# Mehooz/vision4leg

Measured on AMD Instinct MI355X. Metric: PPO env-steps/s (encoder+update, sim excluded), higher is better.
Workload: dtype f16; 1 GPU; ppo_locotransformer thin-goal: LocoTransformer S=93 A=6, E=32 envs x T=512, B=1024, 3 opt epochs; net=loco, envs_per_gpu=32, horizon=512, minibatch=1024, opt_epochs=3, parallelism=dp1, includes_rollout_inference=True, logp_old=recorded at action time (target_pf forward skipped; SURVEY 8d declared saving)

## Files before the change

### vision4leg_amd/csrc/bwd.h

```cpp
#pragma once
#include "infer.h"

namespace v4l {

struct BwdLayer {
  const void *w2t, *w1t, *wot, *wint;
  const float *g1, *g2;
  const float* dy;
  const float *s_qkv, *s_P, *s_xh1, *s_rs1, *s_xh2, *s_rs2;
  const void* s_f;
  void *o_dz2, *o_df, *o_dz1, *o_dqkv;
  float* o_dx;
  float *gp2, *bp2, *gp1, *bp1;
};

struct BwdLayerStack { BwdLayer l[2]; };

struct BwdHead {
  const void *w2t, *w1t, *w0t;
  const float* dout;
  const float *s_h1, *s_h0;
  float *o_dh1, *o_dh0;
};
struct BwdTail {
  const void *wpt, *wf2t, *wupt;
  const float* x0;
  const float *s_e1, *s_e0;
  const float* s_c3;
  float *o_dhc, *o_de0;
  float* o_dc3;
};

template <typename T, int SPW> struct BwdLayLds {
  static constexpr int ROWS = InfRows<SPW>::ROWS;
// ... 656 lines not shown
#pragma unroll
      for (int j = 0; j < 4; ++j) {
        const int n4 = nt4[j] * 16 + qr;
        const float d0 = m[j].x > 0.f ? acc[0][j][0] : 0.f, d1 = m[j].y > 0.f ? acc[0][j][1] : 0.f;
        const float d2 = m[j].z > 0.f ? acc[0][j][2] : 0.f, d3 = m[j].w > 0.f ? acc[0][j][3] : 0.f;
        if (dst != nullptr) st4(dst + fr * LY::LDF + n4, d0, d1, d2, d3);
        if (ok) st4(save + (int64_t)(s0 + fr) * 256 + n4, d0, d1, d2, d3);
      }
    };
    zero_acc(acc);
    block_gemm<T, 1, 4, 2>(acc, dt, LY::LDX, (const T*)tl.wpt, 64, nt4, lane, ring_pr);
    masked(tm_e1, dh, tl.o_dhc);
    __syncthreads();
    zero_acc(acc);
    block_gemm<T, 1, 4, 8>(acc, dh, LY::LDF, (const T*)tl.wf2t, 256, nt4, lane, ring_f2);
    masked(tm_e0, (T*)nullptr, tl.o_de0);
  }
  LAY_STAMP(9);
}


struct BwdConv {
  const void* w3d;
  const void* w2d[4];
  const void* image;
  const int* rowidx;
  const float *c1, *c2;
  const float* dc3;
  float *slab1, *slab2, *slab3;
  float *bslab1, *bslab2, *bslab3;
  int n;
  void *t_dc2, *t_dc1;
};
template <typename T> struct BwdConvLds {
  static constexpr bool B16 = sizeof(T) == 2;
  static constexpr int LF = 64 + 4;
  static constexpr int LC1 = 32 + (B16 ? 8 : 0);
  static constexpr int IMGP = B16 ? 1 : 2;
  static constexpr int LT = 64 + (B16 ? 8 : 4);
  static constexpr int LP2 = 64 + (B16 ? 8 : 4);
  static constexpr int LP1 = 256 + (B16 ? 8 : 4);
  static constexpr size_t dc3_b = (size_t)17 * LT * sizeof(T);
  static constexpr size_t c2_b = (size_t)36 * LF * 4;
  static constexpr size_t dc2_b = (size_t)48 * LT * sizeof(T);
  static constexpr size_t dc2T_b = (size_t)64 * LP2 * sizeof(T);
  static constexpr size_t c1_b = ((size_t)225 * LC1 * sizeof(T) + 15) / 16 * 16;
  static constexpr size_t dc1_b = (size_t)32 * LP1 * sizeof(T);
  static constexpr size_t img_b = (size_t)(4 / IMGP) * 4096 * sizeof(T);
  static constexpr size_t w2_b = B16 ? (size_t)4 * 32 * 256 * sizeof(T) : 0;
  static constexpr size_t bytes = dc3_b + c2_b + dc2_b + dc2T_b + c1_b + dc1_b + img_b + w2_b;
  static_assert(bytes <= 160 * 1024, "one block per CU");
};

template <typename T> __device__ __forceinline__ typename Frag<T>::type frag_of(const float (&v)[8]) {
  typename Frag<T>::type f;
  if constexpr (sizeof(T) == 2) {
#pragma unroll
    for (int j = 0; j < 8; ++j) f[j] = (T)v[j];
  } else {
#pragma unroll
    for (int j = 0; j < 8; ++j) f.v[j] = v[j];
  }
  return f;
}
template <typename H>
__device__ __forceinline__ typename Frag<H>::type frag_of_t(const H (&v)[8]) {
  static_assert(sizeof(H) == 2, "16-bit operand type");
  typename Frag<H>::type f;
#pragma unroll
  for (int j = 0; j < 8; ++j) f[j] = v[j];
  return f;
}
__device__ __forceinline__ f32x8 frag_of_t(const float (&v)[8]) { return frag_of<float>(v); }

template <typename T, int MT, int NT, int KS, int KS0 = 0, int PDEPTH = 4, class RowF>
__device__ __forceinline__ void gather_gemm(f32x4 (&acc)[MT][NT], const T* __restrict__ W, int Kp, int nt0, int lane, RowF arow) {
  typedef typename Frag<T>::type frag_t;
  constexpr int PD = NT >= 2 ? 2 : (KS < PDEPTH ? KS : PDEPTH);
  const int fr = lane & 15, fg = (lane >> 4) * 8;
  const T* wrow = W + (int64_t)(nt0 * 16 + fr) * Kp + fg + KS0 * 32;
  frag_t fb[PD][NT];
#pragma unroll
  for (int d = 0; d < PD; ++d)
#pragma unroll
    for (int j = 0; j < NT; ++j) fb[d][j] = *reinterpret_cast<const frag_t*>(wrow + (int64_t)j * 16 * Kp + d * 32);
#pragma unroll
  for (int ks = 0; ks < KS; ++ks) {
    frag_t cur[NT];
#pragma unroll
    for (int j = 0; j < NT; ++j) cur[j] = fb[ks % PD][j];
    if (ks + PD < KS) {
#pragma unroll
      for (int j = 0; j < NT; ++j) fb[ks % PD][j] = *reinterpret_cast<const frag_t*>(wrow + (int64_t)j * 16 * Kp + (ks + PD) * 32);
    }
#pragma unroll
    for (int mt = 0; mt < MT; ++mt) {
      const frag_t fa = *reinterpret_cast<const frag_t*>(arow(mt, (ks + KS0) >> 1) + ((ks + KS0) & 1) * 32 + fg);
#pragma unroll
      for (int j = 0; j < NT; ++j)
        mma_k32(acc[mt][j], cur[j], fa);
    }
  }
}

#ifdef V4L_INFER_TIMING
#define CONV_STAMP(i) do { if (blockIdx.x == 0 && threadIdx.x == 0 && smp == 3 * (int)gridDim.x) g_inf_stamps[16 + (i)] = clock64(); } while (0)
#else
#define CONV_STAMP(i)
#endif
template <typename T, bool A16 = false>
__global__ __launch_bounds__(512) void bwd_conv_kernel(BwdConv a) {
  static_assert(!A16 || sizeof(T) == 2, "A16: activations saved in the bf16 operand type");
  typedef BwdConvLds<T> LY;
  typedef typename Frag<T>::type frag_t;
  constexpr int NTH = 512;
  extern __shared__ __attribute__((aligned(16))) unsigned char smem[];
  T* sdc3 = reinterpret_cast<T*>(smem);
  float* sc2 = reinterpret_cast<float*>(smem + LY::dc3_b);
  T* sdc2t = reinterpret_cast<T*>(smem + LY::dc3_b + LY::c2_b);
  T* sdc2T = reinterpret_cast<T*>(smem + LY::dc3_b + LY::c2_b + LY::dc2_b);
  constexpr size_t o_c1 = LY::dc3_b + LY::c2_b + LY::dc2_b + LY::dc2T_b;
  T* sc1 = reinterpret_cast<T*>(smem + o_c1);
  T* sdc1T = reinterpret_cast<T*>(smem + o_c1 + LY::c1_b);
  T* simg = reinterpret_cast<T*>(smem + o_c1 + LY::c1_b + LY::dc1_b);
  T* sw2 = reinterpret_cast<T*>(smem + o_c1 + LY::c1_b + LY::dc1_b + LY::img_b);
  const int tid = threadIdx.x, lane = tid & 63, wave = tid >> 6;
  const int fr = lane & 15, g = lane >> 4, qr = g * 4;
  const int kt2 = wave * 4;
  const int ch1 = wave >> 1, th1 = wave & 1;
  f32x4 acc2[4][4], acc1[2][2];
#pragma unroll
  for (int t = 0; t < 4; ++t) {
#pragma unroll
    for (int c = 0; c < 4; ++c) acc2[t][c] = f32x4{0.f, 0.f, 0.f, 0.f};
    acc1[t >> 1][t & 1] = f32x4{0.f, 0.f, 0.f, 0.f};
  }
  float b2r[4] = {0.f, 0.f, 0.f, 0.f};
  float b1r[4] = {0.f, 0.f, 0.f, 0.f};
  for (int i = tid; i < 12 * LY::LT; i += NTH) sdc2t[36 * LY::LT + i] = (T)0.f;
  for (int i = tid; i < 64 * LY::LP2; i += NTH) sdc2T[i] = (T)0.f;
  for (int i = tid; i < 32 * LY::LP1; i += NTH) sdc1T[i] = (T)0.f;
  for (int i = tid; i < LY::LT; i += NTH) sdc3[16 * LY::LT + i] = (T)0.f;
  constexpr int CH = 4 / LY::IMGP;

  constexpr int V = 16 / sizeof(T);
  constexpr int N4 = 225 * 8, PT = (N4 + NTH - 1) / NTH;
  constexpr int N8 = 225 * 4, PT8 = (N8 + NTH - 1) / NTH;
  typedef typename Frag<T>::type chunk_t;
  float4 hv0 = float4{0.f, 0.f, 0.f, 0.f}, hv1 = hv0, cv[A16 ? 1 : PT];
  chunk_t h16 = {}, c16[A16 ? PT8 : 1] = {};
  auto load_next = [&](int sm) {
    const float* g3 = a.dc3 + (int64_t)sm * 16 * 64;
    if constexpr (A16) {
      const chunk_t* g2 = reinterpret_cast<const chunk_t*>(reinterpret_cast<const T*>(a.c2) + (int64_t)sm * 36 * 64);
      const chunk_t* g1 = reinterpret_cast<const chunk_t*>(reinterpret_cast<const T*>(a.c1) + (int64_t)sm * 225 * 32);
      h16 = g2[tid < 288 ? tid : 0];
      if (tid >= 256) hv1 = *reinterpret_cast<const float4*>(g3 + (tid - 256) * 4);
#pragma unroll
      for (int k = 0; k < PT8; ++k) {
        const int i8 = tid + k * NTH;
        c16[k] = g1[i8 < N8 ? i8 : 0];
      }
    } else {
      const float* g2 = a.c2 + (int64_t)sm * 36 * 64;
      const float* g1 = a.c1 + (int64_t)sm * 225 * 32;
      hv0 = *reinterpret_cast<const float4*>(g2 + tid * 4);
      if (tid >= 256) hv1 = *reinterpret_cast<const float4*>(g3 + (tid - 256) * 4);
      else if (tid < 64) hv1 = *reinterpret_cast<const float4*>(g2 + (512 + tid) * 4);
#pragma unroll
      for (int k = 0; k < PT; ++k) {
        const int i4 = tid + k * NTH;
        cv[k] = *reinterpret_cast<const float4*>(g1 + (i4 < N4 ? i4 : 0) * 4);
      }
    }
// ... 57 lines not shown
        const int px = m * 16 + fr;
        okr[m] = px < 36;
        iy[m] = px / 6; ix[m] = px - iy[m] * 6;
      }
      f32x4 acc[3][1];
#pragma unroll
      for (int m = 0; m < 3; ++m) acc[m][0] = f32x4{0.f, 0.f, 0.f, 0.f};
      auto arow = [&](int m, int tap) -> const T* {
        const int ta = tap / 3, tb = tap - ta * 3;
        const int oy = iy[m] - ta, ox = ix[m] - tb;
        const bool ok = okr[m] && oy >= 0 && oy < 4 && ox >= 0 && ox < 4;
        return sdc3 + (ok ? oy * 4 + ox : 16) * LY::LT;
      };
      float4* part = reinterpret_cast<float4*>(simg);
      if (wave >= 4) {
        gather_gemm<T, 3, 1, 9, 9, LY::B16 ? 9 : 3>(acc, W, 576, nt, lane, arow);
#pragma unroll
        for (int m = 0; m < 3; ++m) part[(nt * 3 + m) * 64 + lane] = float4{acc[m][0][0], acc[m][0][1], acc[m][0][2], acc[m][0][3]};
      } else {
        gather_gemm<T, 3, 1, 9, 0, LY::B16 ? 9 : 3>(acc, W, 576, nt, lane, arow);
      }
      __syncthreads();
      if (wave < 4) {
#pragma unroll
        for (int m = 0; m < 3; ++m) {
          const int px = m * 16 + fr, c4 = nt * 16 + qr;
          if (px < 36) {
            const float4 hi = part[(nt * 3 + m) * 64 + lane];
            const float4 mk = *reinterpret_cast<const float4*>(sc2 + px * LY::LF + c4);
            const float d0 = mk.x > 0.f ? acc[m][0][0] + hi.x : 0.f, d1 = mk.y > 0.f ? acc[m][0][1] + hi.y : 0.f;
            const float d2 = mk.z > 0.f ? acc[m][0][2] + hi.z : 0.f, d3 = mk.w > 0.f ? acc[m][0][3] + hi.w : 0.f;
            st4(sdc2t + px * LY::LT + c4, d0, d1, d2, d3);
            if (a.t_dc2 != nullptr) st4(reinterpret_cast<T*>(a.t_dc2) + ((int64_t)smp * 36 + px) * 64 + c4, d0, d1, d2, d3);
            T* tp = sdc2T + c4 * LY::LP2 + px;
            tp[0] = (T)d0; tp[LY::LP2] = (T)d1; tp[2 * LY::LP2] = (T)d2; tp[3 * LY::LP2] = (T)d3;
            b2r[0] += d0; b2r[1] += d1; b2r[2] += d2; b2r[3] += d3;
          }
        }
      }
    }
    __syncthreads();
    CONV_STAMP(2);
#pragma unroll
    for (int k = 0; k < CH * 4096 / V / NTH; ++k)
      __builtin_amdgcn_global_load_lds((const V4L_GLOBAL void*)(gimg + (int64_t)(tid + k * NTH) * V),
                                       (__attribute__((address_space(3))) void*)(simg + ((tid & ~63) + k * NTH) * V), 16, 0, 0);
#pragma unroll
    for (int st = 0; st < 2; ++st) {
      frag_t fy[4];
#pragma unroll
      for (int c = 0; c < 4; ++c) fy[c] = *reinterpret_cast<const frag_t*>(sdc2T + (c * 16 + fr) * LY::LP2 + st * 32 + g * 8);
#pragma unroll
      for (int t = 0; t < 4; ++t) {
        const int kt = kt2 + t, tap = kt >> 1, ci = (kt & 1) * 16 + fr;
        const int ky = tap >> 2, kx = tap & 3;
        T w[8];
#pragma unroll
        for (int j = 0; j < 8; ++j) {
          const int pos = st * 32 + g * 8 + j;
          const int pp = pos < 36 ? pos : 0, oy = pp / 6, ox = pp - oy * 6;
          w[j] = sc1[((2 * oy + ky) * 15 + 2 * ox + kx) * LY::LC1 + ci];
        }
        const frag_t fx = frag_of_t(w);
#pragma unroll
        for (int c = 0; c < 4; ++c) mma_k32(acc2[t][c], fx, fy[c]);
      }
    }
    CONV_STAMP(3);
    {
      const int cls = wave >> 1, py = cls >> 1, pxx = cls & 1, nh = wave & 1;
      const int nIy = (15 - py + 1) >> 1, nIx = (15 - pxx + 1) >> 1;
      int ry[4], rx[4];
#pragma unroll
      for (int m = 0; m < 4; ++m) { const int r = m * 16 + fr; ry[m] = r >> 3; rx[m] = r & 7; }
      f32x4 acc[4][1];
#pragma unroll
      for (int m = 0; m < 4; ++m) acc[m][0] = f32x4{0.f, 0.f, 0.f, 0.f};
      auto arow = [&](int m, int tap) -> const T* {
        const int oy = ry[m] - (tap >> 1), ox = rx[m] - (tap & 1);
        const bool ok = ry[m] < nIy && rx[m] < nIx && oy >= 0 && oy < 6 && ox >= 0 && ox < 6;
        return sdc2t + (ok ? oy * 6 + ox : 36) * LY::LT;
      };
      if constexpr (LY::B16) {
        const T* wl = sw2 + (cls * 2 + nh) * 8 * 512 + lane * 8;
#pragma unroll
        for (int ks = 0; ks < 8; ++ks) {
          const frag_t fw = *reinterpret_cast<const frag_t*>(wl + ks * 512);
#pragma unroll
          for (int m = 0; m < 4; ++m)
            mma_k32(acc[m][0], fw, *reinterpret_cast<const frag_t*>(arow(m, ks >> 1) + (ks & 1) * 32 + g * 8));
        }
      } else {
        gather_gemm<T, 4, 1, 8>(acc, reinterpret_cast<const T*>(a.w2d[cls]), 256, nh, lane, arow);
      }
#pragma unroll
      for (int m = 0; m < 4; ++m) {
        if (ry[m] < nIy && rx[m] < nIx) {
          const int p = (py + 2 * ry[m]) * 15 + pxx + 2 * rx[m];
          const int c4 = nh * 16 + qr;
          const float4 mk = ld4(sc1 + p * LY::LC1 + c4);
          const float d0 = mk.x > 0.f ? acc[m][0][0] : 0.f, d1 = mk.y > 0.f ? acc[m][0][1] : 0.f;
          const float d2 = mk.z > 0.f ? acc[m][0][2] : 0.f, d3 = mk.w > 0.f ? acc[m][0][3] : 0.f;
          T* tp = sdc1T + c4 * LY::LP1 + p;
          tp[0] = (T)d0; tp[LY::LP1] = (T)d1; tp[2 * LY::LP1] = (T)d2; tp[3 * LY::LP1] = (T)d3;
          if (a.t_dc1 != nullptr) st4(reinterpret_cast<T*>(a.t_dc1) + ((int64_t)smp * 225 + p) * 32 + c4, d0, d1, d2, d3);
          b1r[0] += d0; b1r[1] += d1; b1r[2] += d2; b1r[3] += d3;
        }
      }
    }
    __syncthreads();
    CONV_STAMP(4);
    CONV_STAMP(5);
    const bool more = smp + (int)gridDim.x < a.n;
    if (more) load_next(smp + gridDim.x);
#pragma unroll 1
    for (int h = 0; h < LY::IMGP; ++h) {
      if (h > 0) {
        __syncthreads();
        for (int i = tid; i < CH * 4096 / V; i += NTH)
          *reinterpret_cast<float4*>(simg + i * V) = *reinterpret_cast<const float4*>(gimg + (int64_t)h * CH * 4096 + i * V);
        __syncthreads();
      }
      if (ch1 >= h * CH && ch1 < (h + 1) * CH) {
        const T* ich = simg + (ch1 - h * CH) * 4096;
#pragma unroll 1
        for (int st = 0; st < 8; ++st) {
          frag_t fy[2];
#pragma unroll
          for (int c = 0; c < 2; ++c) fy[c] = *reinterpret_cast<const frag_t*>(sdc1T + (c * 16 + fr) * LY::LP1 + st * 32 + g * 8);
          int po2[8];
#pragma unroll
          for (int j = 0; j < 8; ++j) {
            const int pos = st * 32 + g * 8 + j;
            const int pp = pos < 225 ? pos : 0, oy = pp / 15, ox = pp - oy * 15;
            po2[j] = (4 * oy) * 64 + 4 * ox;
          }
#pragma unroll
          for (int tt = 0; tt < 2; ++tt) {
            const int ky = (th1 * 2 + tt) * 2 + (fr >> 3), kx = fr & 7;
            T w[8];
#pragma unroll
            for (int j = 0; j < 8; ++j) w[j] = ich[po2[j] + ky * 64 + kx];
            const frag_t fx = frag_of_t(w);
#pragma unroll
            for (int c = 0; c < 2; ++c) mma_k32(acc1[c][tt], fx, fy[c]);
          }
        }
      }
    }
    if (more) store_next();
    CONV_STAMP(6);
  }
  {
    float* o2 = a.slab2 + (int64_t)blockIdx.x * 64 * 512;
#pragma unroll
    for (int t = 0; t < 4; ++t)
#pragma unroll
// ... 3 lines not shown
    float* o1 = a.slab1 + (int64_t)blockIdx.x * 32 * 256;
#pragma unroll
    for (int c = 0; c < 2; ++c)
#pragma unroll
      for (int tt = 0; tt < 2; ++tt)
        *reinterpret_cast<float4*>(o1 + (c * 16 + fr) * 256 + (ch1 * 4 + th1 * 2 + tt) * 16 + qr) =
            float4{acc1[c][tt][0], acc1[c][tt][1], acc1[c][tt][2], acc1[c][tt][3]};
    __syncthreads();
    float* red2 = reinterpret_cast<float*>(sdc1T);
    float* red1 = red2 + 64 * 16;
    static_assert(LY::dc1_b >= (64 * 16 + 32 * 64) * 4, "bias reduction scratch");
    if (wave < 4) {
#pragma unroll
      for (int i = 0; i < 4; ++i) red2[((wave & 3) * 16 + qr + i) * 16 + fr] = b2r[i];
    }
#pragma unroll
    for (int i = 0; i < 4; ++i) red1[((wave & 1) * 16 + qr + i) * 64 + (wave >> 1) * 16 + fr] = b1r[i];
    __syncthreads();
    if (tid < 64) {
      float t = 0.f;
#pragma unroll
      for (int k = 0; k < 16; ++k) t += red2[tid * 16 + k];
      a.bslab2[(int64_t)blockIdx.x * 64 + tid] = t;
    }
    if (tid < 32) {
      float t = 0.f;
#pragma unroll 8
      for (int k = 0; k < 64; ++k) t += red1[tid * 64 + k];
      a.bslab1[(int64_t)blockIdx.x * 32 + tid] = t;
    }
  }
}

template <typename T, bool A16 = false>
__global__ __launch_bounds__(256) void bwd_conv3_wgrad_kernel(BwdConv a) {
  typedef typename Frag<T>::type frag_t;
  constexpr int LF = 64 + 4;
  __shared__ __attribute__((aligned(16))) float sdc3[16 * LF];
  __shared__ __attribute__((aligned(16))) float sc2[36 * LF];
  const int tid = threadIdx.x, lane = tid & 63, wave = tid >> 6;
  const int fr = lane & 15, g = lane >> 4, qr = g * 4;
  const int kt3 = wave * 9;
  f32x4 acc3[9][4];
#pragma unroll
  for (int t = 0; t < 9; ++t)
#pragma unroll
    for (int c = 0; c < 4; ++c) acc3[t][c] = f32x4{0.f, 0.f, 0.f, 0.f};
  float bias3 = 0.f;
  int x_base[9], x_pos[8];
#pragma unroll
  for (int t = 0; t < 9; ++t) {
    const int kt = kt3 + t, tap = kt >> 2, ky = tap / 3, kx = tap - ky * 3;
    x_base[t] = (ky * 6 + kx) * LF + (kt & 3) * 16 + fr;
  }
#pragma unroll
  for (int j = 0; j < 8; ++j) {
    const int pos = (g & 1) * 8 + j;
    x_pos[j] = ((pos >> 2) * 6 + (pos & 3)) * LF;
  }
  const int i2 = tid + 512 < 36 * 16 ? tid + 512 : 0;
  float4 r3 = {0.f, 0.f, 0.f, 0.f}, r2a = r3, r2b = r3, r2c = r3;
  typedef typename Frag<T>::type chunk_t;
  chunk_t q2a = {}, q2b = {};
  auto fetch = [&](int sm) {
    const float* g3 = a.dc3 + (int64_t)sm * 16 * 64;
    r3 = *reinterpret_cast<const float4*>(g3 + tid * 4);
    if constexpr (A16) {
      const chunk_t* g2 = reinterpret_cast<const chunk_t*>(reinterpret_cast<const T*>(a.c2) + (int64_t)sm * 36 * 64);
      q2a = g2[tid];
      q2b = g2[tid < 32 ? 256 + tid : 0];
    } else {
      const float* g2 = a.c2 + (int64_t)sm * 36 * 64;
      r2a = *reinterpret_cast<const float4*>(g2 + tid * 4);
      r2b = *reinterpret_cast<const float4*>(g2 + (tid + 256) * 4);
      r2c = *reinterpret_cast<const float4*>(g2 + i2 * 4);
    }
  };
  auto file = [&]() {
    *reinterpret_cast<float4*>(sdc3 + (tid >> 4) * LF + (tid & 15) * 4) = r3;
    if constexpr (A16) {
      auto put = [&](int j, const chunk_t& q) {
        float* d = sc2 + (j >> 3) * LF + (j & 7) * 8;
        *reinterpret_cast<float4*>(d) = float4{(float)q[0], (float)q[1], (float)q[2], (float)q[3]};
        *reinterpret_cast<float4*>(d + 4) = float4{(float)q[4], (float)q[5], (float)q[6], (float)q[7]};
      };
      put(tid, q2a);
      if (tid < 32) put(256 + tid, q2b);
    } else {
      *reinterpret_cast<float4*>(sc2 + (tid >> 4) * LF + (tid & 15) * 4) = r2a;
      *reinterpret_cast<float4*>(sc2 + ((tid + 256) >> 4) * LF + (tid & 15) * 4) = r2b;
      if (tid + 512 < 36 * 16) *reinterpret_cast<float4*>(sc2 + ((tid + 512) >> 4) * LF + (tid & 15) * 4) = r2c;
    }
  };
  if ((int)blockIdx.x < a.n) fetch(blockIdx.x);
  for (int smp = blockIdx.x; smp < a.n; smp += gridDim.x) {
    __syncthreads();
    file();
    const int nxt = smp + (int)gridDim.x;
    if (nxt < a.n) fetch(nxt);
    __syncthreads();
    if (tid < 64) {
      float t = 0.f;
#pragma unroll
      for (int p = 0; p < 16; ++p) t += sdc3[p * LF + tid];
      bias3 += t;
    }
    float v[8];
    frag_t fy[4];
#pragma unroll
    for (int c = 0; c < 4; ++c) {
#pragma unroll
      for (int j = 0; j < 8; ++j) {
        const float x = sdc3[((g & 1) * 8 + j) * LF + c * 16 + fr];
        v[j] = g < 2 ? x : 0.f;
      }
      fy[c] = frag_of<T>(v);
    }
#pragma unroll
    for (int t = 0; t < 9; ++t) {
#pragma unroll
      for (int j = 0; j < 8; ++j) {
        const float x = sc2[x_base[t] + x_pos[j]];
        v[j] = g < 2 ? x : 0.f;
      }
      const frag_t fx = frag_of<T>(v);
#pragma unroll
      for (int c = 0; c < 4; ++c) mma_k32(acc3[t][c], fx, fy[c]);
    }
  }
  float* o3 = a.slab3 + (int64_t)blockIdx.x * 64 * 576;
#pragma unroll
  for (int t = 0; t < 9; ++t)
#pragma unroll
    for (int c = 0; c < 4; ++c)
      *reinterpret_cast<float4*>(o3 + (c * 16 + fr) * 576 + (kt3 + t) * 16 + qr) =
          float4{acc3[t][c][0], acc3[t][c][1], acc3[t][c][2], acc3[t][c][3]};
  if (tid < 64) a.bslab3[(int64_t)blockIdx.x * 64 + tid] = bias3;
}

}
```

### vision4leg_amd/csrc/common.h

```cpp
#pragma once
#include <hip/hip_runtime.h>
#include <stdint.h>
#include <stdio.h>
#include <string.h>

namespace v4l {

typedef __attribute__((ext_vector_type(8))) __bf16 bf16x8;
typedef __attribute__((ext_vector_type(8))) _Float16 f16x8;
typedef __attribute__((ext_vector_type(4))) float f32x4;
template <typename H, int N> struct HVec { typedef H type __attribute__((ext_vector_type(N))); };

void set_error(const char* fmt, ...);
const char* last_error();

#define V4L_HIP_CHECK(...)   \
  do {                                                                             \
    hipError_t _e = (__VA_ARGS__);                                                 \
    if (_e != hipSuccess) {                                                        \
      v4l::set_error("%s:%d: %s -> %s", __FILE__, __LINE__, #__VA_ARGS__,          \
                     hipGetErrorString(_e));                                       \
      return -2;                                                                   \
    }                                                                              \
  } while (0)
// ... 39 lines not shown
template <> struct ModeOf<_Float16> { static constexpr int value = 2; };

template <typename T> __device__ __forceinline__ float rt(float x) { return Op<T>::to_f32(Op<T>::from_f32(x)); }
template <typename T> __device__ __forceinline__ float4 rt4(float4 v) { return float4{rt<T>(v.x), rt<T>(v.y), rt<T>(v.z), rt<T>(v.w)}; }

__device__ __forceinline__ void mma_k32(f32x4& acc, const bf16x8& a, const bf16x8& b) {
  acc = __builtin_amdgcn_mfma_f32_16x16x32_bf16(a, b, acc, 0, 0, 0);
}
__device__ __forceinline__ void mma_k32(f32x4& acc, const f16x8& a, const f16x8& b) {
  acc = __builtin_amdgcn_mfma_f32_16x16x32_f16(a, b, acc, 0, 0, 0);
}
struct __attribute__((aligned(16))) f32x8 { float v[8]; };
__device__ __forceinline__ void mma_k32(f32x4& acc, const f32x8& a, const f32x8& b) {
#ifdef V4L_PROBE_F32_SPLIT3
  bf16x8 ah, al, bh, bl;
#pragma unroll
  for (int j = 0; j < 8; ++j) {
    ah[j] = (__bf16)a.v[j]; al[j] = (__bf16)(a.v[j] - (float)ah[j]);
    bh[j] = (__bf16)b.v[j]; bl[j] = (__bf16)(b.v[j] - (float)bh[j]);
  }
  acc = __builtin_amdgcn_mfma_f32_16x16x32_bf16(al, bh, acc, 0, 0, 0);
  acc = __builtin_amdgcn_mfma_f32_16x16x32_bf16(ah, bl, acc, 0, 0, 0);
  acc = __builtin_amdgcn_mfma_f32_16x16x32_bf16(ah, bh, acc, 0, 0, 0);
#else
#pragma unroll
  for (int j = 0; j < 8; ++j) acc = __builtin_amdgcn_mfma_f32_16x16x4f32(a.v[j], b.v[j], acc, 0, 0, 0);
#endif
}
template <typename T> struct Frag;
template <> struct Frag<__bf16> { typedef bf16x8 type; };
template <> struct Frag<_Float16> { typedef f16x8 type; };
template <> struct Frag<float> { typedef f32x8 type; };

template <typename H>
__device__ __forceinline__ void st4(H* p, float a, float b, float c, float d) {
  static_assert(sizeof(H) == 2, "16-bit operand type");
  typename HVec<H, 4>::type v;
  v[0] = (H)a; v[1] = (H)b; v[2] = (H)c; v[3] = (H)d;
  *reinterpret_cast<typename HVec<H, 4>::type*>(p) = v;
}
__device__ __forceinline__ void st4(float* p, float a, float b, float c, float d) {
  *reinterpret_cast<float4*>(p) = float4{a, b, c, d};
}
template <typename H>
__device__ __forceinline__ float4 ld4(const H* p) {
  static_assert(sizeof(H) == 2, "16-bit operand type");
  const typename HVec<H, 4>::type v = *reinterpret_cast<const typename HVec<H, 4>::type*>(p);
  return float4{(float)v[0], (float)v[1], (float)v[2], (float)v[3]};
}
__device__ __forceinline__ float4 ld4(const float* p) { return *reinterpret_cast<const float4*>(p); }

template <int CTRL> __device__ __forceinline__ float dpp_mov(float v) {
  return __int_as_float(__builtin_amdgcn_update_dpp(0, __float_as_int(v), CTRL, 0xf, 0xf, true));
}
__device__ __forceinline__ float lane_bcast(float v, int lane) {
  return __int_as_float(__builtin_amdgcn_readlane(__float_as_int(v), lane));
}
__device__ __forceinline__ float wave_sum(float v) {
  v += dpp_mov<0x128>(v);
  v += dpp_mov<0x124>(v);
  v += dpp_mov<0x122>(v);
  v += dpp_mov<0x121>(v);
  return (lane_bcast(v, 0) + lane_bcast(v, 16)) + (lane_bcast(v, 32) + lane_bcast(v, 48));
}
__device__ __forceinline__ float wave_max(float v) {
  v = fmaxf(v, dpp_mov<0x128>(v));
// ... 36 lines not shown
```

### vision4leg_amd/csrc/v4l_hip.hip

```cpp
#include <math.h>
#include <stdarg.h>

#include <algorithm>
#include <type_traits>

#include <dlfcn.h>

#include "net.h"
#include "infer.h"
#include "bwd.h"
#include "wps.h"
#include "wps_fb.h"
#include "rollout_dense.h"
#include "dense_stack.h"
#include "host_step.h"

namespace v4l {

static thread_local char g_err[1024] = "";
static bool sw_on(const char* name) { return getenv(name) != nullptr; }
template <typename T> struct TypeTag { typedef T type; };
#ifdef V4L_DEV_ONLY
template <class F> static inline int by_compute(int compute, F&& f) {
  typedef std::conditional<V4L_DEV_ONLY == V4L_BF16, __bf16, std::conditional<V4L_DEV_ONLY == V4L_F16, _Float16, float>::type>::type T;
// ... 140 lines not shown
  return 0;
}

static inline bool capturing(hipStream_t s) {
  hipStreamCaptureStatus st = hipStreamCaptureStatusNone;
  if (s == nullptr || hipStreamIsCapturing(s, &st) != hipSuccess) return false;
  return st != hipStreamCaptureStatusNone;
}
struct TnPlan { int BN, KT, gx, gy, splits, mpb, Npad, Kpad; int64_t slab_floats, bslab_floats; };
static inline TnPlan tn_plan(int M, int N, int Kx, bool bf16) {
  TnPlan p;
  p.BN = N <= 16 ? 16 : (N <= 32 ? 32 : 64);
  p.KT = (Kx >= 256 && bf16 && M >= 4096) ? 4 : (Kx >= 128 ? 2 : 1);
  p.gy = cdiv(N, p.BN);
  p.gx = cdiv(Kx, 64 * p.KT);
  int splits = std::max(1, 1024 / (p.gx * p.gy));
  splits = std::min(splits, std::max(1, M / 256));
  p.mpb = round_up(cdiv(M, splits), 64);
  p.splits = cdiv(M, p.mpb);
  p.Npad = p.gy * p.BN;
  p.Kpad = p.gx * 64 * p.KT;
  p.slab_floats = ((int64_t)p.splits * p.Npad * p.Kpad + 63) / 64 * 64;
  p.bslab_floats = ((int64_t)p.splits * p.Npad + 63) / 64 * 64;
  return p;
}

struct Ctx {
  v4l_net* net;
  hipStream_t s;
  float* grads;
  float* slab;
  int64_t slab_used;
  hipStream_t tn;
  bool defer_conv3 = false, conv3_pending = false, conv3_a16 = false;
  v4l::BwdConv conv3_args = {};
  int conv3_blocks = 0, conv3_n = 0;
  bool wps_pending = false;
  bool wps_used = false;
  v4l::WpsWg wps_args = {};
  bool fb_pending = false;
  v4l::FbLoss fb_args = {};
  int fb_blocks = 0, fb_n = 0;
  bool taps = false;
};

static int par_begin(Ctx& c, bool in_capture_too = false) {
  v4l_net* n = c.net;
  if (n->aux == nullptr || (capturing(c.s) && !in_capture_too)) return 0;
  V4L_TRACE("par_begin net=%p s=%p aux=%p", (void*)n, (void*)c.s, (void*)n->aux);
  V4L_HIP_CHECK(hipEventRecord(n->ev_fork, c.s));
  V4L_HIP_CHECK(hipStreamWaitEvent(n->aux, n->ev_fork, 0));
  c.tn = n->aux;
  return 0;
}
static int par_end(Ctx& c) {
  v4l_net* n = c.net;
  if (n->aux == nullptr || c.tn == c.s) return 0;
  V4L_TRACE("par_end net=%p", (void*)n);
  V4L_HIP_CHECK(hipEventRecord(n->ev_join, n->aux));
  V4L_HIP_CHECK(hipStreamWaitEvent(c.s, n->ev_join, 0));
  c.tn = c.s;
  return 0;
}

template <typename T, class YL, class XL>
static int launch_tn(Ctx& c, const YL& yl, const XL& xl, int M, int N, int Kx, RedDesc rd, double flops) {
  if (M <= 0) return 0;
// ... 317 lines not shown

template <typename T>
static int conv_stack_fwd(const Ctx& c, const T* image, const int* rowidx, int n, float* c1, float* c2, float* c3) {
  const v4l_net* N = c.net;
  const Conv* cv = N->conv;
  int rc;
  {
    Epi ep = mk_epi(c1, cv[0].Cout, cv[0].Cout, N->p[cv[0].b], 1);
    auto al = chw_loader<T>(image, cv[0], n, rowidx);
    g_op = "conv1.fwd";
    rc = launch_nt<T>(c.s, al, al.M, (const T*)N->packed + cv[0].pk, cv[0].Np, cv[0].Kp, ep, 2.0 * al.M * cv[0].Cout * cv[0].K);
    if (rc) return rc;
  }
  float* ins[3] = {nullptr, c1, c2};
  float* outs[3] = {c1, c2, c3};
  for (int i = 1; i < 3; ++i) {
    Epi ep = mk_epi(outs[i], cv[i].Cout, cv[i].Cout, N->p[cv[i].b], 1);
    auto al = nhwc_loader(ins[i], cv[i], n);
    g_op = i == 1 ? "conv2.fwd" : "conv3.fwd";
    rc = launch_nt<T>(c.s, al, al.M, (const T*)N->packed + cv[i].pk, cv[i].Np, cv[i].Kp, ep, 2.0 * al.M * cv[i].Cout * cv[i].K);
    if (rc) return rc;
  }
  return 0;
}

static bool conv_bwd_fusable(const v4l_net* N) {
  const Conv* v = N->conv;
  return v[1].Rd == 32 && v[1].Kdp == 256 && v[2].Rd == 64 && v[2].Kdp == 576 && v[0].chw && v[0].Cin == 4 && v[0].IH == 64 && v[0].KH == 8 && v[0].stride == 4 && v[0].Cout == 32 &&
         v[1].Cin == 32 && v[1].KH == 4 && v[1].stride == 2 && v[1].Cout == 64 && v[1].OH == 6 &&
         v[2].Cin == 64 && v[2].KH == 3 && v[2].stride == 1 && v[2].Cout == 64 && v[2].OH == 4 &&
         !sw_on("V4L_NO_FUSED_CONV_BWD");
}
template <typename T>
static int conv_stack_bwd_fused(Ctx& c, const T* image, const int* rowidx, int n, const float* c1, const float* c2,
                                const float* dc3, float* dc2_tap, float* dc1_tap) {
  v4l_net* N = c.net;
  V4L_HIP_CHECK(lds_limit<&bwd_conv_kernel<T>>(BwdConvLds<T>::bytes));
  if constexpr (sizeof(T) == 2) V4L_HIP_CHECK(lds_limit<&bwd_conv_kernel<T, true>>(BwdConvLds<T>::bytes));
  const bool a16 = sizeof(T) == 2 && N->acts16_c1 != nullptr && N->acts16_c1 == c1;
  int nblk = std::min(n, CONV_BWD_MAX_BLOCKS);
  if (const char* e = getenv("V4L_CONV_BWD_BLOCKS")) nblk = std::max(1, std::min(nblk, atoi(e)));
  int nblk3 = std::min(nblk, c.wps_used ? 96 : 160);
  if (const char* e = getenv("V4L_CONV3_WGRAD_BLOCKS")) nblk3 = std::max(1, std::min(nblk, atoi(e)));
  const int Ns[3] = {32, 64, 64}, Ks[3] = {256, 512, 576};
  float* slab[3];
  float* bslab[3];
  for (int i = 0; i < 3; ++i) {
    const int nb = i == 2 ? nblk3 : nblk;
    const int64_t sf = ((int64_t)nb * Ns[i] * Ks[i] + 63) / 64 * 64, bf = ((int64_t)nb * Ns[i] + 63) / 64 * 64;
    slab[i] = c.slab + c.slab_used;
    bslab[i] = slab[i] + sf;
    c.slab_used += sf + bf;
    const Conv& v = N->conv[i];
    RedDesc o;
    memset(&o, 0, sizeof(o));
    o.dW = c.grads + N->params[v.w].goff;
    o.db = c.grads + N->params[v.b].goff;
    o.N = v.Cout; o.K = v.K; o.Ktorch = v.K;
    o.Cin = v.chw ? 0 : v.Cin; o.taps = v.chw ? 0 : v.KH * v.KH;
    o.slab = slab[i]; o.bslab = bslab[i]; o.nsplit = nb; o.Npad = Ns[i]; o.Kpad = Ks[i];
    o.group = 1;
    N->red.push_back(o);
  }
  V4L_REQUIRE(c.slab_used <= N->slab_cap, "internal: weight-grad slab arena overflow");
  BwdConv a;
  memset(&a, 0, sizeof(a));
  a.w3d = (const T*)N->packed + N->conv[2].pkd[0];
  for (int cls = 0; cls < 4; ++cls) a.w2d[cls] = (const T*)N->packed + N->conv[1].pkd[cls];
  a.image = image; a.rowidx = rowidx; a.c1 = c1; a.c2 = c2; a.dc3 = dc3;
  if (c.taps) { a.t_dc2 = dc2_tap; a.t_dc1 = dc1_tap; }
  a.slab1 = slab[0]; a.slab2 = slab[1]; a.slab3 = slab[2];
  a.bslab1 = bslab[0]; a.bslab2 = bslab[1]; a.bslab3 = bslab[2];
  a.n = n;
  g_op = "conv.bwd";
  const double fl = 2.0 * n * (16.0 * 64 * 576 + 2.0 * 36 * 64 * 512 + 225.0 * 32 * 256);
  if constexpr (sizeof(T) == 2) {
    if (a16) V4L_KLAUNCH("fused_conv_bwd", fl, c.s, (bwd_conv_kernel<T, true>), dim3(nblk), dim3(512), BwdConvLds<T>::bytes, c.s, a);
  }
  if (!a16) V4L_KLAUNCH("fused_conv_bwd", fl, c.s, bwd_conv_kernel<T>, dim3(nblk), dim3(512), BwdConvLds<T>::bytes, c.s, a);
  V4L_LAUNCH_CHECK();
  if (c.defer_conv3) {
    c.conv3_args = a; c.conv3_blocks = nblk3; c.conv3_n = n; c.conv3_pending = true; c.conv3_a16 = a16;
    return 0;
  }
  g_op = "conv3.wgrad";
  if constexpr (sizeof(T) == 2) {
    if (a16) V4L_KLAUNCH("fused_conv3_wgrad", 2.0 * n * 16 * 64 * 576, c.tn, (bwd_conv3_wgrad_kernel<T, true>), dim3(nblk3), dim3(256), 0, c.tn, a);
  }
  if (!a16) V4L_KLAUNCH("fused_conv3_wgrad", 2.0 * n * 16 * 64 * 576, c.tn, bwd_conv3_wgrad_kernel<T>, dim3(nblk3), dim3(256), 0, c.tn, a);
  V4L_LAUNCH_CHECK();
  return 0;
}
template <typename T>
static int conv3_wgrad_deferred(Ctx& c, hipStream_t s) {
  if (!c.conv3_pending) return 0;
  c.conv3_pending = false;
  g_op = "conv3.wgrad";
  if constexpr (sizeof(T) == 2) {
    if (c.conv3_a16)
      V4L_KLAUNCH("fused_conv3_wgrad", 2.0 * c.conv3_n * 16 * 64 * 576, s, (bwd_conv3_wgrad_kernel<T, true>), dim3(c.conv3_blocks),
                  dim3(256), 0, s, c.conv3_args);
  }
  if (!c.conv3_a16)
    V4L_KLAUNCH("fused_conv3_wgrad", 2.0 * c.conv3_n * 16 * 64 * 576, s, bwd_conv3_wgrad_kernel<T>, dim3(c.conv3_blocks), dim3(256), 0, s,
                c.conv3_args);
  V4L_LAUNCH_CHECK();
  return 0;
}

template <typename T>
static int conv_stack_bwd(Ctx& c, const T* image, const int* rowidx, int n, const float* c1, const float* c2,
                          float* dc3, float* dc2, float* dc1) {
  if (conv_bwd_fusable(c.net)) return conv_stack_bwd_fused<T>(c, image, rowidx, n, c1, c2, dc3, dc2, dc1);
  const v4l_net* N = c.net;
  const Conv* cv = N->conv;
  const float* acts[3] = {nullptr, c1, c2};
  float* dys[3] = {dc1, dc2, dc3};
  for (int i = 2; i >= 0; --i) {
    const Conv& v = cv[i];
    const int M = n * v.OH * v.OH;
    ADense y = dense(dys[i], v.Cout, M, v.Cout);
    RedDesc o;
    memset(&o, 0, sizeof(o));
    o.dW = c.grads + N->params[v.w].goff;
    o.db = c.grads + N->params[v.b].goff;
    o.N = v.Cout; o.K = v.K; o.Ktorch = v.K;
    int rc;
    if (i > 0 && (rc = par_begin(c))) return rc;
    if (v.chw) {
      o.Cin = 0; o.taps = 0;
      auto x = chw_loader<T>(image, v, n, rowidx);
      g_op = "conv1.wgrad";
      rc = launch_tn<T>(c, y, x, M, v.Cout, v.K, o, 2.0 * M * v.Cout * v.K);
    } else {
      o.Cin = v.Cin; o.taps = v.KH * v.KH;
      auto x = nhwc_loader(acts[i], v, n);
      g_op = i == 1 ? "conv2.wgrad" : "conv3.wgrad";
      rc = launch_tn<T>(c, y, x, M, v.Cout, v.K, o, 2.0 * M * v.Cout * v.K);
    }
    if (rc) return rc;
// ... 3641 lines not shown
```

Baseline: 402,900 env-steps/s.

## Use ds_read_tr16 transposed LDS reads for conv weight-gradient operands

Adds a 16-bit-only path in the fused conv backward and conv3 wgrad kernels. Operand fragments come from row-major LDS images through ds_read_tr16_b64, with precomputed lane offset maps, instead of building separate transposed LDS copies with scalar scattered stores. This removes the transposed dc2 buffer and the strided transpose writes, and moves the image DMA after the dw2 GEMM. In exchange it adds an offset table in LDS, more complex addressing, and a new code path that is on by default through V4L_WGRAD_TR.

After: 428,100 env-steps/s, median of 6. +6.2%, better.

```diff
diff --git a/vision4leg_amd/csrc/bwd.h b/vision4leg_amd/csrc/bwd.h
--- a/vision4leg_amd/csrc/bwd.h
+++ b/vision4leg_amd/csrc/bwd.h
@@ -1,5 +1,6 @@
 #pragma once
 #include "infer.h"
+#include "tr_maps.h"
 
 namespace v4l {
 
@@ -722,8 +723,9 @@
   int n;
   void *t_dc2, *t_dc1;
 };
-template <typename T> struct BwdConvLds {
+template <typename T, bool TR = false> struct BwdConvLds {
   static constexpr bool B16 = sizeof(T) == 2;
+  static_assert(!TR || B16, "transposed LDS reads are 16-bit only");
   static constexpr int LF = 64 + 4;
   static constexpr int LC1 = 32 + (B16 ? 8 : 0);
   static constexpr int IMGP = B16 ? 1 : 2;
@@ -733,13 +735,18 @@
   static constexpr size_t dc3_b = (size_t)17 * LT * sizeof(T);
   static constexpr size_t c2_b = (size_t)36 * LF * 4;
   static constexpr size_t dc2_b = (size_t)48 * LT * sizeof(T);
-  static constexpr size_t dc2T_b = (size_t)64 * LP2 * sizeof(T);
+  static constexpr size_t dc2T_b = TR ? 0 : (size_t)64 * LP2 * sizeof(T);
   static constexpr size_t c1_b = ((size_t)225 * LC1 * sizeof(T) + 15) / 16 * 16;
-  static constexpr size_t dc1_b = (size_t)32 * LP1 * sizeof(T);
+  static constexpr int LD1 = 32 + 8;
+  static constexpr size_t dc1_b = (size_t)(TR ? 256 * LD1 : 32 * LP1) * sizeof(T);
   static constexpr size_t img_b = (size_t)(4 / IMGP) * 4096 * sizeof(T);
   static constexpr size_t w2_b = B16 ? (size_t)4 * 32 * 256 * sizeof(T) : 0;
-  static constexpr size_t bytes = dc3_b + c2_b + dc2_b + dc2T_b + c1_b + dc1_b + img_b + w2_b;
+  static constexpr size_t tab_b = TR ? (size_t)8 * 64 * 4 : 0;
+  static constexpr size_t bytes = dc3_b + c2_b + dc2_b + dc2T_b + c1_b + dc1_b + img_b + w2_b + tab_b;
   static_assert(bytes <= 160 * 1024, "one block per CU");
+  static_assert(!TR || (LC1 == trmap::LC1 && LT == trmap::LT && LD1 == trmap::LD1), "tr_maps.h describes these rows");
+  static_assert((dc3_b + c2_b) % 16 == 0 && (dc3_b + c2_b + dc2_b + dc2T_b) % 16 == 0 && c1_b % 16 == 0 && dc1_b % 16 == 0,
+                "every image starts on a 16-byte boundary (transposed reads: 8)");
 };
 
 template <typename T> __device__ __forceinline__ typename Frag<T>::type frag_of(const float (&v)[8]) {
@@ -798,10 +805,10 @@
 #else
 #define CONV_STAMP(i)
 #endif
-template <typename T, bool A16 = false>
+template <typename T, bool A16 = false, bool TR = false>
 __global__ __launch_bounds__(512) void bwd_conv_kernel(BwdConv a) {
   static_assert(!A16 || sizeof(T) == 2, "A16: activations saved in the bf16 operand type");
-  typedef BwdConvLds<T> LY;
+  typedef BwdConvLds<T, TR> LY;
   typedef typename Frag<T>::type frag_t;
   constexpr int NTH = 512;
   extern __shared__ __attribute__((aligned(16))) unsigned char smem[];
@@ -814,6 +821,7 @@
   T* sdc1T = reinterpret_cast<T*>(smem + o_c1 + LY::c1_b);
   T* simg = reinterpret_cast<T*>(smem + o_c1 + LY::c1_b + LY::dc1_b);
   T* sw2 = reinterpret_cast<T*>(smem + o_c1 + LY::c1_b + LY::dc1_b + LY::img_b);
+  uint32_t* stab = reinterpret_cast<uint32_t*>(smem + o_c1 + LY::c1_b + LY::dc1_b + LY::img_b + LY::w2_b);
   const int tid = threadIdx.x, lane = tid & 63, wave = tid >> 6;
   const int fr = lane & 15, g = lane >> 4, qr = g * 4;
   const int kt2 = wave * 4;
@@ -828,8 +836,19 @@
   float b2r[4] = {0.f, 0.f, 0.f, 0.f};
   float b1r[4] = {0.f, 0.f, 0.f, 0.f};
   for (int i = tid; i < 12 * LY::LT; i += NTH) sdc2t[36 * LY::LT + i] = (T)0.f;
-  for (int i = tid; i < 64 * LY::LP2; i += NTH) sdc2T[i] = (T)0.f;
-  for (int i = tid; i < 32 * LY::LP1; i += NTH) sdc1T[i] = (T)0.f;
+  if constexpr (!TR) {
+    for (int i = tid; i < 64 * LY::LP2; i += NTH) sdc2T[i] = (T)0.f;
+  }
+  for (int i = tid; i < (int)(LY::dc1_b / sizeof(T)); i += NTH) sdc1T[i] = (T)0.f;
+  int a2o[2][2] = {{0, 0}, {0, 0}};
+  if constexpr (TR) {
+#pragma unroll
+    for (int st = 0; st < 2; ++st)
+#pragma unroll
+      for (int h = 0; h < 2; ++h) a2o[st][h] = trmap::dw2_a_lane(st, lane, h);
+    for (int i = tid; i < 8 * 64; i += NTH)
+      stab[i] = (uint32_t)trmap::dw1_a_lane(i >> 6, i & 63, 0) | (uint32_t)trmap::dw1_a_lane(i >> 6, i & 63, 1) << 16;
+  }
   for (int i = tid; i < LY::LT; i += NTH) sdc3[16 * LY::LT + i] = (T)0.f;
   constexpr int CH = 4 / LY::IMGP;
 
@@ -953,8 +972,10 @@
             const float d2 = mk.z > 0.f ? acc[m][0][2] + hi.z : 0.f, d3 = mk.w > 0.f ? acc[m][0][3] + hi.w : 0.f;
             st4(sdc2t + px * LY::LT + c4, d0, d1, d2, d3);
             if (a.t_dc2 != nullptr) st4(reinterpret_cast<T*>(a.t_dc2) + ((int64_t)smp * 36 + px) * 64 + c4, d0, d1, d2, d3);
-            T* tp = sdc2T + c4 * LY::LP2 + px;
-            tp[0] = (T)d0; tp[LY::LP2] = (T)d1; tp[2 * LY::LP2] = (T)d2; tp[3 * LY::LP2] = (T)d3;
+            if constexpr (!TR) {
+              T* tp = sdc2T + c4 * LY::LP2 + px;
+              tp[0] = (T)d0; tp[LY::LP2] = (T)d1; tp[2 * LY::LP2] = (T)d2; tp[3 * LY::LP2] = (T)d3;
+            }
             b2r[0] += d0; b2r[1] += d1; b2r[2] += d2; b2r[3] += d3;
           }
         }
@@ -962,13 +983,30 @@
     }
     __syncthreads();
     CONV_STAMP(2);
-#pragma unroll
-    for (int k = 0; k < CH * 4096 / V / NTH; ++k)
-      __builtin_amdgcn_global_load_lds((const V4L_GLOBAL void*)(gimg + (int64_t)(tid + k * NTH) * V),
-                                       (__attribute__((address_space(3))) void*)(simg + ((tid & ~63) + k * NTH) * V), 16, 0, 0);
+    auto image_dma = [&]() {
+#pragma unroll
+      for (int k = 0; k < CH * 4096 / V / NTH; ++k)
+        __builtin_amdgcn_global_load_lds((const V4L_GLOBAL void*)(gimg + (int64_t)(tid + k * NTH) * V),
+                                         (__attribute__((address_space(3))) void*)(simg + ((tid & ~63) + k * NTH) * V), 16, 0, 0);
+    };
+    if constexpr (!TR) image_dma();
 #pragma unroll
     for (int st = 0; st < 2; ++st) {
       frag_t fy[4];
+      if constexpr (TR) {
+        const T* pb0 = sdc2t + trmap::dw2_b_lane(st, lane, 0);
+        const T* pb1 = sdc2t + trmap::dw2_b_lane(st, lane, 1);
+#pragma unroll
+        for (int c = 0; c < 4; ++c) fy[c] = frag_tr(pb0 + c * 16, pb1 + c * 16);
+#pragma unroll
+        for (int t = 0; t < 4; ++t) {
+          const T* pa = sc1 + trmap::dw2_a_tile(kt2 + t);
+          const frag_t fx = frag_tr(pa + a2o[st][0], pa + a2o[st][1]);
+#pragma unroll
+          for (int c = 0; c < 4; ++c) mma_k32(acc2[t][c], fx, fy[c]);
+        }
+        continue;
+      }
 #pragma unroll
       for (int c = 0; c < 4; ++c) fy[c] = *reinterpret_cast<const frag_t*>(sdc2T + (c * 16 + fr) * LY::LP2 + st * 32 + g * 8);
 #pragma unroll
@@ -987,6 +1025,7 @@
         for (int c = 0; c < 4; ++c) mma_k32(acc2[t][c], fx, fy[c]);
       }
     }
+    if constexpr (TR) image_dma();
     CONV_STAMP(3);
     {
       const int cls = wave >> 1, py = cls >> 1, pxx = cls & 1, nh = wave & 1;
@@ -1022,8 +1061,12 @@
           const float4 mk = ld4(sc1 + p * LY::LC1 + c4);
           const float d0 = mk.x > 0.f ? acc[m][0][0] : 0.f, d1 = mk.y > 0.f ? acc[m][0][1] : 0.f;
           const float d2 = mk.z > 0.f ? acc[m][0][2] : 0.f, d3 = mk.w > 0.f ? acc[m][0][3] : 0.f;
-          T* tp = sdc1T + c4 * LY::LP1 + p;
-          tp[0] = (T)d0; tp[LY::LP1] = (T)d1; tp[2 * LY::LP1] = (T)d2; tp[3 * LY::LP1] = (T)d3;
+          if constexpr (TR) {
+            st4(sdc1T + p * LY::LD1 + c4, d0, d1, d2, d3);
+          } else {
+            T* tp = sdc1T + c4 * LY::LP1 + p;
+            tp[0] = (T)d0; tp[LY::LP1] = (T)d1; tp[2 * LY::LP1] = (T)d2; tp[3 * LY::LP1] = (T)d3;
+          }
           if (a.t_dc1 != nullptr) st4(reinterpret_cast<T*>(a.t_dc1) + ((int64_t)smp * 225 + p) * 32 + c4, d0, d1, d2, d3);
           b1r[0] += d0; b1r[1] += d1; b1r[2] += d2; b1r[3] += d3;
         }
@@ -1044,6 +1087,27 @@
       }
       if (ch1 >= h * CH && ch1 < (h + 1) * CH) {
         const T* ich = simg + (ch1 - h * CH) * 4096;
+        if constexpr (TR) {
+          const T* pb0 = sdc1T + trmap::dw1_b_lane(0, lane, 0);
+          const T* pb1 = sdc1T + trmap::dw1_b_lane(0, lane, 1);
+#pragma unroll 4
+          for (int st = 0; st < 8; ++st) {
+            const uint32_t po = stab[st * 64 + lane];
+            const T* pa0 = ich + (po & 0xffffu);
+            const T* pa1 = ich + (po >> 16);
+            frag_t fy[2];
+#pragma unroll
+            for (int c = 0; c < 2; ++c) fy[c] = frag_tr(pb0 + st * 32 * LY::LD1 + c * 16, pb1 + st * 32 * LY::LD1 + c * 16);
+#pragma unroll
+            for (int tt = 0; tt < 2; ++tt) {
+              const int ot = trmap::dw1_a_tile(th1 * 2 + tt);
+              const frag_t fx = frag_tr(pa0 + ot, pa1 + ot);
+#pragma unroll
+              for (int c = 0; c < 2; ++c) mma_k32(acc1[c][tt], fx, fy[c]);
+            }
+          }
+          continue;
+        }
 #pragma unroll 1
         for (int st = 0; st < 8; ++st) {
           frag_t fy[2];
@@ -1113,12 +1177,15 @@
   }
 }
 
-template <typename T, bool A16 = false>
+template <typename T, bool A16 = false, bool TR = false>
 __global__ __launch_bounds__(256) void bwd_conv3_wgrad_kernel(BwdConv a) {
+  static_assert(!TR || sizeof(T) == 2, "transposed LDS reads are 16-bit only");
   typedef typename Frag<T>::type frag_t;
-  constexpr int LF = 64 + 4;
+  constexpr int LF = 64 + 4, L3 = trmap::L3;
   __shared__ __attribute__((aligned(16))) float sdc3[16 * LF];
-  __shared__ __attribute__((aligned(16))) float sc2[36 * LF];
+  __shared__ __attribute__((aligned(16))) float sc2[TR ? 4 : 36 * LF];
+  __shared__ __attribute__((aligned(16))) T sdc3t[TR ? 17 * L3 : 8];
+  __shared__ __attribute__((aligned(16))) T sc2t[TR ? trmap::C2R * L3 : 8];
   const int tid = threadIdx.x, lane = tid & 63, wave = tid >> 6;
   const int fr = lane & 15, g = lane >> 4, qr = g * 4;
   const int kt3 = wave * 9;
@@ -1159,7 +1226,17 @@
   };
   auto file = [&]() {
     *reinterpret_cast<float4*>(sdc3 + (tid >> 4) * LF + (tid & 15) * 4) = r3;
-    if constexpr (A16) {
+    if constexpr (TR) {
+      st4(sdc3t + (tid >> 4) * L3 + (tid & 15) * 4, r3.x, r3.y, r3.z, r3.w);
+      if constexpr (A16) {
+        *reinterpret_cast<chunk_t*>(sc2t + (tid >> 3) * L3 + (tid & 7) * 8) = q2a;
+        if (tid < 32) *reinterpret_cast<chunk_t*>(sc2t + ((256 + tid) >> 3) * L3 + (tid & 7) * 8) = q2b;
+      } else {
+        st4(sc2t + (tid >> 4) * L3 + (tid & 15) * 4, r2a.x, r2a.y, r2a.z, r2a.w);
+        st4(sc2t + ((tid + 256) >> 4) * L3 + (tid & 15) * 4, r2b.x, r2b.y, r2b.z, r2b.w);
+        if (tid + 512 < 36 * 16) st4(sc2t + ((tid + 512) >> 4) * L3 + (tid & 15) * 4, r2c.x, r2c.y, r2c.z, r2c.w);
+      }
+    } else if constexpr (A16) {
       auto put = [&](int j, const chunk_t& q) {
         float* d = sc2 + (j >> 3) * LF + (j & 7) * 8;
         *reinterpret_cast<float4*>(d) = float4{(float)q[0], (float)q[1], (float)q[2], (float)q[3]};
@@ -1173,6 +1250,12 @@
       if (tid + 512 < 36 * 16) *reinterpret_cast<float4*>(sc2 + ((tid + 512) >> 4) * LF + (tid & 15) * 4) = r2c;
     }
   };
+  const int b3o[2] = {trmap::dw3_b_lane(lane, 0), trmap::dw3_b_lane(lane, 1)};
+  const int a3o[2] = {trmap::dw3_a_lane(lane, 0), trmap::dw3_a_lane(lane, 1)};
+  if constexpr (TR) {
+    for (int i = tid; i < L3; i += 256) sdc3t[16 * L3 + i] = (T)0.f;
+    for (int i = tid; i < (trmap::C2R - 36) * L3; i += 256) sc2t[36 * L3 + i] = (T)0.f;
+  }
   if ((int)blockIdx.x < a.n) fetch(blockIdx.x);
   for (int smp = blockIdx.x; smp < a.n; smp += gridDim.x) {
     __syncthreads();
@@ -1188,6 +1271,18 @@
     }
     float v[8];
     frag_t fy[4];
+    if constexpr (TR) {
+#pragma unroll
+      for (int c = 0; c < 4; ++c) fy[c] = frag_tr(sdc3t + b3o[0] + c * 16, sdc3t + b3o[1] + c * 16);
+#pragma unroll
+      for (int t = 0; t < 9; ++t) {
+        const T* pa = sc2t + trmap::dw3_a_tile(kt3 + t);
+        const frag_t fx = frag_tr(pa + a3o[0], pa + a3o[1]);
+#pragma unroll
+        for (int c = 0; c < 4; ++c) mma_k32(acc3[t][c], fx, fy[c]);
+      }
+      continue;
+    }
 #pragma unroll
     for (int c = 0; c < 4; ++c) {
 #pragma unroll
diff --git a/vision4leg_amd/csrc/common.h b/vision4leg_amd/csrc/common.h
--- a/vision4leg_amd/csrc/common.h
+++ b/vision4leg_amd/csrc/common.h
@@ -95,6 +95,16 @@
 template <> struct Frag<_Float16> { typedef f16x8 type; };
 template <> struct Frag<float> { typedef f32x8 type; };
 
+typedef short s16x4_t __attribute__((vector_size(8)));
+template <typename H>
+__device__ __forceinline__ typename Frag<H>::type frag_tr(const H* p0, const H* p1) {
+  static_assert(sizeof(H) == 2, "16-bit operand type");
+  typedef __attribute__((address_space(3))) s16x4_t* lds_p;
+  const s16x4_t lo = __builtin_amdgcn_ds_read_tr16_b64_v4i16((lds_p)p0);
+  const s16x4_t hi = __builtin_amdgcn_ds_read_tr16_b64_v4i16((lds_p)p1);
+  return __builtin_bit_cast(typename Frag<H>::type, __builtin_shufflevector(lo, hi, 0, 1, 2, 3, 4, 5, 6, 7));
+}
+
 template <typename H>
 __device__ __forceinline__ void st4(H* p, float a, float b, float c, float d) {
   static_assert(sizeof(H) == 2, "16-bit operand type");
diff --git a/vision4leg_amd/csrc/tr_maps.h b/vision4leg_amd/csrc/tr_maps.h
--- /dev/null
+++ b/vision4leg_amd/csrc/tr_maps.h
@@ -0,0 +1,54 @@
+#pragma once
+#if defined(__HIPCC__)
+#define V4L_TRMAP __host__ __device__ constexpr
+#else
+#define V4L_TRMAP constexpr
+#endif
+
+namespace v4l {
+namespace trmap {
+
+constexpr int LC1 = 40;
+constexpr int LT = 72;
+constexpr int LD1 = 40;
+constexpr int L3 = 72;
+constexpr int C2R = 36 + 15;
+
+V4L_TRMAP int tr_k(int lane, int h) { return 8 * (lane >> 4) + 4 * h + ((lane & 15) >> 2); }
+V4L_TRMAP int tr_c(int lane) { return 4 * (lane & 3); }
+
+V4L_TRMAP int dw2_a_lane(int st, int lane, int h) {
+  const int pos = st * 32 + tr_k(lane, h), pp = pos < 36 ? pos : 0, oy = pp / 6, ox = pp - oy * 6;
+  return (2 * oy * 15 + 2 * ox) * LC1 + tr_c(lane);
+}
+V4L_TRMAP int dw2_a_tile(int kt) {
+  const int tap = kt >> 1, ky = tap >> 2, kx = tap & 3;
+  return (ky * 15 + kx) * LC1 + (kt & 1) * 16;
+}
+V4L_TRMAP int dw2_b_lane(int st, int lane, int h) {
+  const int pos = st * 32 + tr_k(lane, h);
+  return (pos < 36 ? pos : 36) * LT + tr_c(lane);
+}
+
+V4L_TRMAP int dw1_a_lane(int st, int lane, int h) {
+  const int pos = st * 32 + tr_k(lane, h), pp = pos < 225 ? pos : 0, oy = pp / 15, ox = pp - oy * 15, p = lane & 3;
+  return (4 * oy + (p >> 1)) * 64 + 4 * ox + 4 * (p & 1);
+}
+V4L_TRMAP int dw1_a_tile(int kyt) { return 2 * kyt * 64; }
+V4L_TRMAP int dw1_b_lane(int st, int lane, int h) { return (st * 32 + tr_k(lane, h)) * LD1 + tr_c(lane); }
+
+V4L_TRMAP int dw3_a_lane(int lane, int h) {
+  const int pos = tr_k(lane, h);
+  return (pos < 16 ? (pos >> 2) * 6 + (pos & 3) : 36) * L3 + tr_c(lane);
+}
+V4L_TRMAP int dw3_a_tile(int kt) {
+  const int tap = kt >> 2, ky = tap / 3, kx = tap - ky * 3;
+  return (ky * 6 + kx) * L3 + (kt & 3) * 16;
+}
+V4L_TRMAP int dw3_b_lane(int lane, int h) {
+  const int pos = tr_k(lane, h);
+  return (pos < 16 ? pos : 16) * L3 + tr_c(lane);
+}
+
+}
+}
diff --git a/vision4leg_amd/csrc/v4l_hip.hip b/vision4leg_amd/csrc/v4l_hip.hip
--- a/vision4leg_amd/csrc/v4l_hip.hip
+++ b/vision4leg_amd/csrc/v4l_hip.hip
@@ -196,7 +196,7 @@
   float* slab;
   int64_t slab_used;
   hipStream_t tn;
-  bool defer_conv3 = false, conv3_pending = false, conv3_a16 = false;
+  bool defer_conv3 = false, conv3_pending = false, conv3_a16 = false, conv3_tr = false;
   v4l::BwdConv conv3_args = {};
   int conv3_blocks = 0, conv3_n = 0;
   bool wps_pending = false;
@@ -580,14 +580,35 @@
          !sw_on("V4L_NO_FUSED_CONV_BWD");
 }
 template <typename T>
+static int conv3_wgrad_launch(Ctx& c, hipStream_t s) {
+  g_op = "conv3.wgrad";
+  const double fl = 2.0 * c.conv3_n * 16 * 64 * 576;
+  const dim3 grid(c.conv3_blocks), blk(256);
+  const bool a16 = c.conv3_a16, tr = c.conv3_tr;
+  if constexpr (sizeof(T) == 2) {
+    if (a16 && tr) V4L_KLAUNCH("fused_conv3_wgrad", fl, s, (bwd_conv3_wgrad_kernel<T, true, true>), grid, blk, 0, s, c.conv3_args);
+    else if (a16) V4L_KLAUNCH("fused_conv3_wgrad", fl, s, (bwd_conv3_wgrad_kernel<T, true>), grid, blk, 0, s, c.conv3_args);
+    else if (tr) V4L_KLAUNCH("fused_conv3_wgrad", fl, s, (bwd_conv3_wgrad_kernel<T, false, true>), grid, blk, 0, s, c.conv3_args);
+  }
+  if (!a16 && !tr) V4L_KLAUNCH("fused_conv3_wgrad", fl, s, bwd_conv3_wgrad_kernel<T>, grid, blk, 0, s, c.conv3_args);
+  V4L_LAUNCH_CHECK();
+  return 0;
+}
+template <typename T>
 static int conv_stack_bwd_fused(Ctx& c, const T* image, const int* rowidx, int n, const float* c1, const float* c2,
                                 const float* dc3, float* dc2_tap, float* dc1_tap) {
   v4l_net* N = c.net;
   V4L_HIP_CHECK(lds_limit<&bwd_conv_kernel<T>>(BwdConvLds<T>::bytes));
-  if constexpr (sizeof(T) == 2) V4L_HIP_CHECK(lds_limit<&bwd_conv_kernel<T, true>>(BwdConvLds<T>::bytes));
+  if constexpr (sizeof(T) == 2) {
+    V4L_HIP_CHECK(lds_limit<&bwd_conv_kernel<T, true>>(BwdConvLds<T>::bytes));
+    V4L_HIP_CHECK(lds_limit<&bwd_conv_kernel<T, false, true>>(BwdConvLds<T, true>::bytes));
+    V4L_HIP_CHECK(lds_limit<&bwd_conv_kernel<T, true, true>>(BwdConvLds<T, true>::bytes));
+  }
   const bool a16 = sizeof(T) == 2 && N->acts16_c1 != nullptr && N->acts16_c1 == c1;
   int nblk = std::min(n, CONV_BWD_MAX_BLOCKS);
   if (const char* e = getenv("V4L_CONV_BWD_BLOCKS")) nblk = std::max(1, std::min(nblk, atoi(e)));
+  const int tr_sw = sizeof(T) == 2 ? sw_int("V4L_WGRAD_TR", 1) : 0;
+  const bool tr = tr_sw == 1 || tr_sw == 2, tr3 = tr_sw == 1 || tr_sw == 3;
   int nblk3 = std::min(nblk, c.wps_used ? 96 : 160);
   if (const char* e = getenv("V4L_CONV3_WGRAD_BLOCKS")) nblk3 = std::max(1, std::min(nblk, atoi(e)));
   const int Ns[3] = {32, 64, 64}, Ks[3] = {256, 512, 576};
@@ -623,37 +644,24 @@
   g_op = "conv.bwd";
   const double fl = 2.0 * n * (16.0 * 64 * 576 + 2.0 * 36 * 64 * 512 + 225.0 * 32 * 256);
   if constexpr (sizeof(T) == 2) {
-    if (a16) V4L_KLAUNCH("fused_conv_bwd", fl, c.s, (bwd_conv_kernel<T, true>), dim3(nblk), dim3(512), BwdConvLds<T>::bytes, c.s, a);
-  }
-  if (!a16) V4L_KLAUNCH("fused_conv_bwd", fl, c.s, bwd_conv_kernel<T>, dim3(nblk), dim3(512), BwdConvLds<T>::bytes, c.s, a);
-  V4L_LAUNCH_CHECK();
+    if (a16 && tr) V4L_KLAUNCH("fused_conv_bwd", fl, c.s, (bwd_conv_kernel<T, true, true>), dim3(nblk), dim3(512), (BwdConvLds<T, true>::bytes), c.s, a);
+    else if (a16) V4L_KLAUNCH("fused_conv_bwd", fl, c.s, (bwd_conv_kernel<T, true>), dim3(nblk), dim3(512), BwdConvLds<T>::bytes, c.s, a);
+    else if (tr) V4L_KLAUNCH("fused_conv_bwd", fl, c.s, (bwd_conv_kernel<T, false, true>), dim3(nblk), dim3(512), (BwdConvLds<T, true>::bytes), c.s, a);
+  }
+  if (!a16 && !tr) V4L_KLAUNCH("fused_conv_bwd", fl, c.s, bwd_conv_kernel<T>, dim3(nblk), dim3(512), BwdConvLds<T>::bytes, c.s, a);
+  V4L_LAUNCH_CHECK();
+  c.conv3_args = a; c.conv3_blocks = nblk3; c.conv3_n = n; c.conv3_a16 = a16; c.conv3_tr = tr3;
   if (c.defer_conv3) {
-    c.conv3_args = a; c.conv3_blocks = nblk3; c.conv3_n = n; c.conv3_pending = true; c.conv3_a16 = a16;
+    c.conv3_pending = true;
     return 0;
   }
-  g_op = "conv3.wgrad";
-  if constexpr (sizeof(T) == 2) {
-    if (a16) V4L_KLAUNCH("fused_conv3_wgrad", 2.0 * n * 16 * 64 * 576, c.tn, (bwd_conv3_wgrad_kernel<T, true>), dim3(nblk3), dim3(256), 0, c.tn, a);
-  }
-  if (!a16) V4L_KLAUNCH("fused_conv3_wgrad", 2.0 * n * 16 * 64 * 576, c.tn, bwd_conv3_wgrad_kernel<T>, dim3(nblk3), dim3(256), 0, c.tn, a);
-  V4L_LAUNCH_CHECK();
-  return 0;
+  return conv3_wgrad_launch<T>(c, c.tn);
 }
 template <typename T>
 static int conv3_wgrad_deferred(Ctx& c, hipStream_t s) {
   if (!c.conv3_pending) return 0;
   c.conv3_pending = false;
-  g_op = "conv3.wgrad";
-  if constexpr (sizeof(T) == 2) {
-    if (c.conv3_a16)
-      V4L_KLAUNCH("fused_conv3_wgrad", 2.0 * c.conv3_n * 16 * 64 * 576, s, (bwd_conv3_wgrad_kernel<T, true>), dim3(c.conv3_blocks),
-                  dim3(256), 0, s, c.conv3_args);
-  }
-  if (!c.conv3_a16)
-    V4L_KLAUNCH("fused_conv3_wgrad", 2.0 * c.conv3_n * 16 * 64 * 576, s, bwd_conv3_wgrad_kernel<T>, dim3(c.conv3_blocks), dim3(256), 0, s,
-                c.conv3_args);
-  V4L_LAUNCH_CHECK();
-  return 0;
+  return conv3_wgrad_launch<T>(c, s);
 }
 
 template <typename T>
```
